# fatimp/SIFT3D

Hardware: AMD Instinct MI355X
Metric: Mvoxel/s detect+describe (float32 volume resident in HBM) (higher is better)
Workload: dtype f32; 1 GPU; 512x512x512 float32 lattice-blob volume, detect+describe, default parameters (sigma0 1.6, sigma_n 1.15, 3 levels/octave); parallelism=single GPU

## Files before the change

profiles/describe_model.py:

```python
#!/usr/bin/env python3
import csv
import glob
import json
import os
import sys

ROOT = os.path.dirname(os.path.dirname(os.path.abspath(__file__)))
sys.path.insert(0, ROOT)


def _require_built():
    lib = os.environ.get("SIFT3D_AMD_LIB") or os.path.join(ROOT, "sift3d_amd", "libsift3d_amd.so")
    if not os.path.exists(lib):
        sys.exit("%s is missing -- build first: python3 -c \"from sift3d_amd import _native; "
                 "_native.build()\"" % lib)


def run_guarded(*a, **k):
    _require_built()
    return run(*a, **k)


def run(n=512):
    import torch
    from sift3d_amd import api, hip
    vol = torch.empty((n, n, n), device="cuda")
    hip.synth_lattice(vol, 0, 11)
    det, kp, desc = api.Detector(), api.KeypointStore(), api.DescriptorStore()
    assert det.detect_keypoints_device(vol.data_ptr(), n, n, n, kp) == 0
    assert det.extract_descriptors(kp, desc) == 0
    return det, kp, desc


def count():
    import ctypes as C
    from sift3d_amd import api
    L = api.lib()
    L.sift3d_amd_diag_desc_voxels.restype = C.c_ulonglong
    L.sift3d_amd_diag_desc_voxels()
    _require_built()
    det, kp, desc = run()
    print(json.dumps(dict(window_voxels=int(L.sift3d_amd_diag_desc_voxels()), keypoints=len(kp))))


def parse(d, voxels):
    agg = {}
    for f in glob.glob(os.path.join(d, "**", "*counter_collection.csv"), recursive=True):
        for r in csv.DictReader(open(f)):
            if "k_describe" in r["Kernel_Name"]:
                agg.setdefault(r["Counter_Name"], []).append(float(r["Counter_Value"]))
    c = {k: sum(v) / len(v) for k, v in agg.items()}
    out = dict(kernel="k_describe", workload="512^3 lattice volume, 42 501 keypoints", window_voxels=int(voxels),
               valu_insts=c.get("SQ_INSTS_VALU"), salu_insts=c.get("SQ_INSTS_SALU"),
               lds_insts=c.get("SQ_INSTS_LDS"), lds_array_cycles=c.get("SQ_LDS_IDX_ACTIVE"),
               lds_bank_conflict_cycles=c.get("SQ_LDS_BANK_CONFLICT"), waves=c.get("SQ_WAVES"),
               wave_quad_cycles=c.get("SQ_WAVE_CYCLES"), wait_any=c.get("SQ_WAIT_ANY"),
               wait_inst_any=c.get("SQ_WAIT_INST_ANY"), wait_inst_lds=c.get("SQ_WAIT_INST_LDS"),
               note="wave-instructions per launch (rocprofv3 --pmc); lds_array_cycles is summed over the 256 CUs; "
                    "bench.py prices both against the kernel's own cycle count of its run (clock probe)")
    if voxels and c.get("SQ_INSTS_VALU"):
        out["valu_insts_per_64_voxels"] = round(64.0 * c["SQ_INSTS_VALU"] / voxels, 1)
        out["lds_insts_per_64_voxels"] = round(64.0 * c.get("SQ_INSTS_LDS", 0) / voxels, 1)
        out["lds_array_cycles_per_64_voxels"] = round(64.0 * c.get("SQ_LDS_IDX_ACTIVE", 0) / voxels, 1)
    if c.get("SQ_WAVE_CYCLES") and c.get("SQ_WAVES"):
        kc = 4.0 * c["SQ_WAVE_CYCLES"] / c["SQ_WAVES"]
        out["profiled_kernel_cycles"] = round(kc)
        out["lds_array_busy"] = round(c.get("SQ_LDS_IDX_ACTIVE", 0) / (256.0 * kc), 4)
        out["valu_busy"] = round(2.0 * c.get("SQ_INSTS_VALU", 0) / (1024.0 * kc), 4)
        if c.get("GRBM_GUI_ACTIVE"):
            out["grbm_gui_active_cycles"] = c["GRBM_GUI_ACTIVE"]
    print(json.dumps(out, indent=1))


if __name__ == "__main__":
    if "--run" in sys.argv:
        run_guarded()
    elif "--count" in sys.argv:
        count()
    elif "--parse" in sys.argv:
        i = sys.argv.index("--parse")
        parse(sys.argv[i + 1], float(sys.argv[i + 2]))
```

sift3d_amd/csrc/sift3d_describe.hip:

```cpp
#include "sift3d_kernels_common.h"
#include "sift3d_math.h"

#include <algorithm>
#include <cmath>
#include <cstdlib>

struct FaceRec {
    float v0[3], e1[3], e2[3], t[3], q[3], e2q, idx[3];
};
static_assert(sizeof(FaceRec) == SIFT3D_HIP_FACE_FLOATS * 4, "face record layout");

__constant__ float c_face16[20 * 16];
__constant__ int c_bin_off[12];
__constant__ int c_oct_face[32];

constexpr int DQ = 256;
constexpr int HIST_USED = 800;
constexpr int HIST_LDS = 800;
constexpr int FACE_STRIDE = 20;
constexpr int RSUPER = 68;
constexpr int REC_FLOATS = 7 * RSUPER;
constexpr int rec_row(int r) { return r < 7 ? r * RSUPER : (r - 7) * RSUPER + 32; }
constexpr int rec_group(int r) { return (rec_row(r) / 4) % 16; }
constexpr bool rec_groups_distinct()
{
    for (int a = 0; a < 14; a++)
        for (int b = a + 1; b < 14; b++)
            if (rec_group(a) == rec_group(b))
                return false;
    return true;
}
static_assert(rec_groups_distinct(), "record rows: X (0..10) and bin-address rows (11..13) on disjoint bank groups");
static_assert(RSUPER % 4 == 0 && RSUPER >= 64, "record rows: 16-byte aligned, 64 lanes per super-row");

__device__ __forceinline__ uint32_t lds_addr(const void *p)
{
    return (uint32_t)(uintptr_t)(const __attribute__((address_space(3))) void *)p;
}

#ifdef SIFT3D_AMD_DIAG
#define DESC_ABLATE_ARG , int ablate
#define DESC_ABLATE(bit) (ablate & (bit))
__device__ unsigned long long g_desc_voxels;
#else
#define DESC_ABLATE_ARG
#define DESC_ABLATE(bit) false
#endif

__device__ __forceinline__ void wave_sync()
{
    __builtin_amdgcn_fence(__ATOMIC_RELEASE, "wavefront");
    __builtin_amdgcn_wave_barrier();
    __builtin_amdgcn_fence(__ATOMIC_ACQUIRE, "wavefront");
}

__device__ __forceinline__ float quad_fmac(float acc, float x)
{
    asm("v_fmac_f32_dpp %0, %1, %1 quad_perm:[3,0,0,0] row_mask:0xf bank_mask:0xf bound_ctrl:1"
        : "+v"(acc)
        : "v"(x));
    return acc;
}

__device__ __forceinline__ bool face_eval(const float4 *__restrict__ fr, float rx, float ry, float rz,
                                          float &xb, float &yb, float &zb, int &fi)
{
    const float4 A0 = fr[0], A1 = fr[1], A2 = fr[2], A3 = fr[3];
    const float px = ry * A1.y - rz * A1.x;
    const float py = rz * A0.w - rx * A1.y;
    const float pz = rx * A1.x - ry * A0.w;
    const float det = A0.x * px + A0.y * py + A0.z * pz;
    const float di = 1.0f / det;
    yb = di * (A1.z * px + A1.w * py + A2.x * pz);
    zb = di * (rx * A2.y + ry * A2.z + rz * A2.w);
    xb = 1.0f - yb - zb;
    const float kk = A3.x * di;
    fi = __float_as_int(A3.y);
    return !(fabsf(det) < 1.1920928955078125e-06f) &&
           !(xb < -1.1920928955078125e-06f || yb < -1.1920928955078125e-06f ||
             zb < -1.1920928955078125e-06f || kk < 0);
}

__device__ __forceinline__ int icos_guess(float rx, float ry, float rz)
{
    const float g = 1.6180339887f, g2 = 2.6180339887f;
    const float ax = fabsf(rx), ay = fabsf(ry), az = fabsf(rz);
    const float t1 = ax + g2 * ay - g * az;
    const float t2 = ay + g2 * az - g * ax;
    const float t3 = az + g2 * ax - g * ay;
    const int n1 = t1 < 0.0f, n2 = t2 < 0.0f, n3 = t3 < 0.0f;
    const int cls = n1 + (1 - n1) * (2 * n2 + (1 - n2) * 3 * n3);
    return cls * 8 + (int)(rx < 0.0f) + 2 * (int)(ry < 0.0f) + 4 * (int)(rz < 0.0f);
}

constexpr int WL_STRIDE = 4096, WL_HEAD = 4;
constexpr int WL_COUNTERS = 16;

__global__ __launch_bounds__(256) void k_desc_wlut(const sift3d_hip_level *__restrict__ levels, int nlevels,
                                                   float *__restrict__ lut)
{
    const int t = blockIdx.x;
    if (t >= nlevels)
        return;
    if (t == 0 && threadIdx.x < WL_COUNTERS)
        reinterpret_cast<uint32_t *>(lut + (size_t)nlevels * WL_STRIDE)[threadIdx.x] = 0u;
    const sift3d_hip_level L = levels[t];
    float *tab = lut + (size_t)t * WL_STRIDE;
    const float sigma = (float)(L.sd * 7.071067812);
    const float rad = (float)(2.0 * (double)sigma);
    const float rad2 = rad * rad, sig2 = sigma * sigma;
    int e;
    const float mant = frexpf(L.ux, &e);
    const float u2 = L.ux * L.ux;
    const bool ok = L.ux == L.uy && L.ux == L.uz && mant == 0.5f &&
                    rad2 / u2 < (float)(WL_STRIDE - WL_HEAD - 1) && u2 * (float)WL_STRIDE < 16777216.0f;
    if (threadIdx.x == 0) {
        tab[0] = ok ? 1.0f : 0.0f;
        tab[1] = 0.0f;
        tab[2] = __int_as_float((int)(__double_as_longlong(L.sd) & 0xffffffffll));
        tab[3] = __int_as_float((int)(__double_as_longlong(L.sd) >> 32));
    }
    if (!ok)
        return;
    for (int k = threadIdx.x; k < WL_STRIDE - WL_HEAD; k += 256) {
        const float sq = (float)k * u2;
        const float arg = -0.5f * sq / sig2;
// ... 39 lines not shown
    if (probe) {
        probe_c0 = clock64();
        probe_w0 = wall_clock64();
    }
    const bool split = !EXACT && part != nullptr;
    for (bool first_pass = true;; first_pass = false) {
    uint32_t item;
    if (work) {
        uint32_t t = 0;
        if (lane == 0)
            t = atomicAdd(work, 1u);
        item = (uint32_t)__builtin_amdgcn_readfirstlane((int)t);
    } else {
        if (!first_pass)
            break;
        item = blockIdx.x * DWAVES + wv;
    }
    const uint32_t ki = first + (split ? item / DPARTS : item);
    const int pp = split ? (int)(item % DPARTS) : 0;
    if (ki >= n)
        break;
    static_assert(2 * HIST_LDS == 25 * 64, "histogram clear: 25 whole-wave stores");
#define Z4(o) "ds_write_addtid_b32 %0 offset:" #o "\n\tds_write_addtid_b32 %0 offset:" #o "+256\n\t" \
              "ds_write_addtid_b32 %0 offset:" #o "+512\n\tds_write_addtid_b32 %0 offset:" #o "+768\n\t"
    asm volatile("s_mov_b32 m0, %1\n\ts_nop 0\n\t" Z4(0) Z4(1024) Z4(2048) Z4(3072) Z4(4096) Z4(5120)
                 "ds_write_addtid_b32 %0 offset:6144" ::"v"(0.0f), "s"(hist_m0) : "m0", "memory");
#undef Z4
    wave_sync();
    const sift3d_hip_kp K = kps[ki];
    const sift3d_hip_level L = levels[K.level];
    const uint32_t orow = K.row1 ? K.row1 - 1 : ki;
    const float *__restrict__ wtab = nullptr;
    const int icx = (int)K.cx, icy = (int)K.cy, icz = (int)K.cz;
    if (LATTICE) {
        wtab = wlut + (size_t)K.level * WL_STRIDE + WL_HEAD;
    } else if (wlut) {
        const float *tab = wlut + (size_t)K.level * WL_STRIDE;
        const long long sdbits = ((long long)__float_as_int(tab[3]) << 32) | (unsigned)__float_as_int(tab[2]);
        if (tab[0] == 1.0f && sdbits == __double_as_longlong(K.sd) && (float)icx == K.cx &&
            (float)icy == K.cy && (float)icz == K.cz)
            wtab = tab + WL_HEAD;
    }

    typedef const float __attribute__((address_space(1))) *gfloat_p;
    const bool have_tab = LATTICE || wtab;
    const gfloat_p wsrc = have_tab ? (gfloat_p)wtab : (gfloat_p) reinterpret_cast<const float *>(levels);
    const int wmask = have_tab ? -1 : 0;

    const float sigma = (float)(K.sd * 7.071067812);
    const float rad = (float)(2.0 * (double)sigma);
    const float half_w = (float)((double)rad / 1.4142135623730951);
    const float desc_w = 2.0f * half_w;
    const float hist_w = desc_w / 4.0f;
    const float bin_f = 1.0f / hist_w;
    const float rad2 = rad * rad;
    const float sig2 = sigma * sigma;
    const float *R = K.R;
    const float iux = 1.0f / L.ux, iuy = 1.0f / L.uy, iuz = 1.0f / L.uz;
    Box B;
    bounds_f(K.cx, rad, L.ux, L.nx, B.xs, B.xe);
    bounds_f(K.cy, rad, L.uy, L.ny, B.ys, B.ye);
    bounds_f(K.cz, rad, L.uz, L.nz_glob, B.zs, B.ze);
    B.zs = max(B.zs, L.z_off + 1);
    B.ze = min(B.ze, L.z_off + L.nz - 2);
    const int xsh = 32 - __builtin_clz((unsigned)max(B.xe - B.xs, 1));
    const int ysh = xsh + 32 - __builtin_clz((unsigned)max(B.ye - B.ys, 1));
    const uint32_t xmask = (1u << xsh) - 1u, ymask = (1u << (ysh - xsh)) - 1u;
#if defined(__HIP_DEVICE_COMPILE__) && !defined(__gfx942__) && !defined(__gfx950__)
#error "k_describe's commit routes its factors with DPP quad_perm on wave64: validated on gfx942 / gfx950 only"
#endif
    const int half = lane >> 5, l5 = lane & 31;
    const int pc = l5 >> 2, pt = l5 & 3, pj = pt < 3 ? pt : 0;
    const int pxr = pt == 0 ? pc : 8 + pj;
    const int pdx = (pc >> 2) & 1, pdy = (pc >> 1) & 1, pdz = pc & 1;
    const int corner4 = 4 * (pdx + 4 * pdy + 16 * pdz);
    const int coff_a = corner4 + (EXACT ? (half == 0 ? 0 : HIST_LDS * 4) : half * (HIST_LDS * 4));
    const int coff_b = corner4 + (half == 1 ? 0 : HIST_LDS * 4);
    (void)coff_b;

    uint32_t qhead = 0, qtail = 0;
    bool pend = false;
#ifdef SIFT3D_AMD_DIAG
    unsigned diag_voxels = 0;
#endif

    auto window = [&](int x, int y, int z, float &sq, float &vbx, float &vby, float &vbz) -> bool {
        const float dx = ((float)x - K.cx) * L.ux;
        const float dy = ((float)y - K.cy) * L.uy;
        const float dz = ((float)z - K.cz) * L.uz;
        sq = dx * dx + dy * dy + dz * dz;
        const float kx = R[0] * dx + R[3] * dy + R[6] * dz;
        const float ky = R[1] * dx + R[4] * dy + R[7] * dz;
        const float kz = R[2] * dx + R[5] * dy + R[8] * dz;
        vbx = (kx + half_w) * bin_f;
        vby = (ky + half_w) * bin_f;
        vbz = (kz + half_w) * bin_f;
        const float lo = fminf(fminf(vbx, vby), vbz), hi = fmaxf(fmaxf(vbx, vby), vbz);
        return !(sq > rad2) && !(lo < 0.0f) && !(hi >= 4.0f);
    };

    float pv[7] = { 0.f, 0.f, 0.f, 0.f, 0.f, 0.f, 0.f };
    int ppk = 0;
    int pwi = 0, pwj = 0, pwl = 0;
    const gfloat_p gdata = (gfloat_p)L.data;
    const uint32_t ys32 = (uint32_t)L.nx, zs32 = (uint32_t)L.nx * (uint32_t)L.ny;
    auto prefetch_loads = [&](uint32_t start, int cnt) {
        const int qv = queue[(start + lane) & (DQ - 1)];
        ppk = lane < cnt ? qv : ppk;
        const int x = B.xs + (int)((uint32_t)ppk & xmask), y = B.ys + (int)(((uint32_t)ppk >> xsh) & ymask),
                  zl = B.zs + (int)((uint32_t)ppk >> ysh) - L.z_off;
        const gfloat_p p = gdata + ((uint64_t)zs32 * (uint32_t)zl + (uint32_t)(x + (int)ys32 * y));
        pv[0] = p[1]; pv[1] = *(p - 1); pv[2] = p[ys32]; pv[3] = *(p - ys32);
        pv[4] = p[zs32]; pv[5] = *(p - zs32);
        if (wtab) {
            const int i = x - icx, j = y - icy, l = B.zs + (int)((uint32_t)ppk >> ysh) - icz;
            pv[6] = wtab[i * i + j * j + l * l];
            pwi = i; pwj = j; pwl = l;
        }
    };
    auto prefetch_weight = [&]() {
        if (LATTICE || wtab)
            return;
        const int x = B.xs + (int)((uint32_t)ppk & xmask), y = B.ys + (int)(((uint32_t)ppk >> xsh) & ymask);
        const float dx = ((float)x - K.cx) * L.ux;
        const float dy = ((float)y - K.cy) * L.uy;
        const float dz = ((float)(B.zs + (int)((uint32_t)ppk >> ysh)) - K.cz) * L.uz;
        pv[6] = s3d_expf_in_range(-0.5f * (dx * dx + dy * dy + dz * dz) / sig2, sexp);
    };
    auto prefetch = [&](uint32_t start, int cnt) {
        prefetch_loads(start, cnt);
        prefetch_weight();
    };

    float rp[2][7] = { { 0.f, 0.f, 0.f, 0.f, 0.f, 0.f, 0.f }, { 0.f, 0.f, 0.f, 0.f, 0.f, 0.f, 0.f } };
    const float *const xrd = rec + rec_row(pxr) + 16 * half;
    const int *const ard = reinterpret_cast<const int *>(rec + rec_row(11 + pj) + 16 * half);
    auto commit_write = [&](int pass) {
#define RS(i) "ds_write_addtid_b32 %" #i " offset:%c8*" #i "\n\t"
        asm volatile("s_mov_b32 m0, %7\n\ts_nop 0\n\t" RS(0) RS(1) RS(2) RS(3) RS(4) RS(5) RS(6)
                     ::"v"(rp[pass][0]), "v"(rp[pass][1]), "v"(rp[pass][2]), "v"(rp[pass][3]), "v"(rp[pass][4]),
                       "v"(rp[pass][5]), "v"(rp[pass][6]), "s"(rec_m0), "n"(RSUPER * 4)
                     : "m0", "memory");
#undef RS
        wave_sync();
    };
#define SB() __builtin_amdgcn_sched_barrier(0)
#ifndef DESC_OPT
#define DESC_OPT 111
#endif
#define QUAD_X(v) __int_as_float(__builtin_amdgcn_update_dpp(0, __float_as_int(v), 0x03, 0xf, 0xf, true))
#if DESC_OPT & 1
#define COMMIT_ADD(old, x) (EXACT ? (old) + QUAD_X(x) * (x) : quad_fmac(old, x))
#else
#define COMMIT_ADD(old, x) ((old) + QUAD_X(x) * (x))
#endif
#define KEEP(v) asm volatile("" ::"v"(v))
#if (DESC_OPT & 64)
typedef __attribute__((address_space(3))) float *lds_float_p;
#define LDS_F32(a) (*(lds_float_p)(uintptr_t)(uint32_t)(a))
#define OFFCHAIN (!EXACT)
#define CHUNK_ADDR(q)                                                                         \
    aq_[q] = make_int4(bq_[q].x + coffh, bq_[q].y + coffh, bq_[q].z + coffh, bq_[q].w + coffh); \
    KEEP(aq_[q].x); KEEP(aq_[q].y); KEEP(aq_[q].z); KEEP(aq_[q].w);
#define COMMIT_BEGIN(coff)                                                                    \
    const int coffh = (coff) + (int)lds_addr(hist);                                           \
    int4 bq_[2], aq_[2];                                                                      \
    float4 xq_[2];                                                                            \
    bq_[0] = *reinterpret_cast<const int4 *>(ard);                                            \
    xq_[0] = *reinterpret_cast<const float4 *>(xrd);                                          \
    bq_[1] = bq_[0];                                                                          \
    xq_[1] = xq_[0];                                                                          \
    CHUNK_ADDR(0)                                                                             \
    aq_[1] = aq_[0];
#define ROUND(u, ...)                                                                         \
    {                                                                                         \
        constexpr int cur_ = ((u) >> 2) & 1, nxt_ = cur_ ^ 1;                                 \
        const int mb_[4] = { bq_[cur_].x, bq_[cur_].y, bq_[cur_].z, bq_[cur_].w };            \
        const int ma_[4] = { aq_[cur_].x, aq_[cur_].y, aq_[cur_].z, aq_[cur_].w };            \
        const float xv_[4] = { xq_[cur_].x, xq_[cur_].y, xq_[cur_].z, xq_[cur_].w };          \
        const int addr_ = OFFCHAIN ? ma_[(u) & 3] : mb_[(u) & 3] + coffh;                     \
        float old_ = 0.0f;                                                                    \
        if (!DESC_ABLATE(1))                                                                  \
            old_ = LDS_F32(addr_);                                                            \
        SB();                                                                                 \
        if (((u) & 3) == 0 && (u) + 4 < 16) {                                                 \
            bq_[nxt_] = *reinterpret_cast<const int4 *>(ard + (u) + 4);                       \
            xq_[nxt_] = *reinterpret_cast<const float4 *>(xrd + (u) + 4);                     \
            SB();                                                                             \
        }                                                                                     \
        { __VA_ARGS__ }                                                                       \
        if (OFFCHAIN && ((u) & 3) == 1 && (u) + 3 < 16) {                                     \
            CHUNK_ADDR(nxt_)                                                                  \
        }                                                                                     \
        SB();                                                                                 \
        if (!DESC_ABLATE(1))                                                                  \
            LDS_F32(addr_) = COMMIT_ADD(old_, xv_[(u) & 3]);            \
        SB();                                                                                 \
    }
#else
#define COMMIT_BEGIN(coff)                                                                    \
    const int coff4 = (coff);                                                                 \
    int4 cb4 = *reinterpret_cast<const int4 *>(ard);                                          \
    float4 cx4 = *reinterpret_cast<const float4 *>(xrd);                                      \
    int4 nb4 = cb4;                                                                           \
    float4 nx4 = cx4;
#define ROUND(u, ...)                                                                         \
    {                                                                                         \
        if (((u) & 3) == 0 && (u) + 4 < 16) {                                                 \
            nb4 = *reinterpret_cast<const int4 *>(ard + (u) + 4);                             \
            nx4 = *reinterpret_cast<const float4 *>(xrd + (u) + 4);                           \
        }                                                                                     \
        const int mb_[4] = { cb4.x, cb4.y, cb4.z, cb4.w };                                    \
        const float xv_[4] = { cx4.x, cx4.y, cx4.z, cx4.w };                                  \
        float *bin_ = reinterpret_cast<float *>(reinterpret_cast<char *>(hist) + (mb_[(u) & 3] + coff4)); \
        float old_ = 0.0f;                                                                    \
        if (!DESC_ABLATE(1))                                                                  \
            old_ = *bin_;                                                                     \
        SB();                                                                                 \
        { __VA_ARGS__ }                                                                       \
        SB();                                                                                 \
        if (!DESC_ABLATE(1))                                                                  \
            *bin_ = COMMIT_ADD(old_, xv_[(u) & 3]);                     \
        if (((u) & 3) == 3) {                                                                 \
            cb4 = nb4;                                                                        \
            cx4 = nx4;                                                                        \
        }                                                                                     \
        SB();                                                                                 \
    }
#endif
#define CHAIN_B()                                                                             \
    if (EXACT) {                                                                              \
// ... 92 lines not shown
            float mag, fx, fy, fz;
            int ix, iy, iz, cell4;
            float ax[2], ay[2], az[2], fld[14];
            ROUND(0, qv_ = queue[(nstart + lane) & (DQ - 1)];)
            ROUND(1, ppk = lane < ncnt ? qv_ : ppk;
                     nx_ = B.xs + (int)((uint32_t)ppk & xmask); ny_ = B.ys + (int)(((uint32_t)ppk >> xsh) & ymask);
                     nzl_ = B.zs + (int)((uint32_t)ppk >> ysh) - L.z_off;
                     np_ = gdata + ((uint64_t)zs32 * (uint32_t)nzl_ + (uint32_t)(nx_ + (int)ys32 * ny_));)
            ROUND(2, pv[0] = np_[1]; pv[1] = *(np_ - 1); pv[2] = np_[ys32]; pv[3] = *(np_ - ys32);)
            ROUND(3, pv[4] = np_[zs32]; pv[5] = *(np_ - zs32);
                     const int i = nx_ - icx; const int j = ny_ - icy; const int l = B.zs + (int)((uint32_t)ppk >> ysh) - icz;
                     pv[6] = wsrc[(i * i + j * j + l * l) & wmask];
                     if (LATTICE && (DESC_OPT & 8)) { pwi = i; pwj = j; pwl = l; })
#if DESC_OPT & 2
            ROUND(4, mag = EXACT ? sqrtf(m2) : __builtin_amdgcn_sqrtf(m2);
                     mag = live && found ? mag : 0.0f;)
#else
            ROUND(4, mag = sqrtf(m2); mag = live && found ? mag : 0.0f;)
#endif
            ROUND(5, fx = vbx - floorf(vbx); fy = vby - floorf(vby); fz = vbz - floorf(vbz);
                     ix = (int)vbx; iy = (int)vby; iz = (int)vbz;)
            ROUND(6, const bool lx = ix >= 3; const bool ly = iy >= 3; const bool lz = iz >= 3;
                     ax[0] = lx ? 0.0f : 1.0f - fx; ax[1] = lx ? 1.0f - fx : fx;
                     ay[0] = ly ? 0.0f : 1.0f - fy; ay[1] = ly ? 1.0f - fy : fy;
                     az[0] = lz ? 0.0f : 1.0f - fz; az[1] = lz ? 1.0f - fz : fz;)
            ROUND(7, _Pragma("unroll") for (int c = 0; c < 4; c++)
                         fld[c] = mag * (ax[(c >> 2) & 1] * ay[(c >> 1) & 1] * az[c & 1]);)
            ROUND(8, _Pragma("unroll") for (int c = 4; c < 8; c++)
                         fld[c] = mag * (ax[(c >> 2) & 1] * ay[(c >> 1) & 1] * az[c & 1]);)
            ROUND(9, cell4 = 4 * (min(max(ix, 0), 2) + 4 * min(max(iy, 0), 2) + 16 * min(max(iz, 0), 2));
                     const bool ok = live && found;
                     fld[8] = ok ? b0 : 0.0f; fld[9] = ok ? b1 : 0.0f; fld[10] = ok ? b2 : 0.0f;)
            ROUND(10, _Pragma("unroll") for (int j = 0; j < 3; j++)
                          fld[11 + j] = __int_as_float(4 * ((fidx >> (10 * j)) & 1023) + cell4);)
            ROUND(11, _Pragma("unroll") for (int i = 0; i < 4; i++) {
                          const auto r = __builtin_amdgcn_permlane32_swap(__float_as_uint(fld[i]), __float_as_uint(fld[7 + i]), false, false);
                          rp[0][i] = __uint_as_float(r[0]); rp[1][i] = __uint_as_float(r[1]); })
            ROUND(12, _Pragma("unroll") for (int i = 4; i < 7; i++) {
                          const auto r = __builtin_amdgcn_permlane32_swap(__float_as_uint(fld[i]), __float_as_uint(fld[7 + i]), false, false);
                          rp[0][i] = __uint_as_float(r[0]); rp[1][i] = __uint_as_float(r[1]); })
            ROUND(13, )
            ROUND(14, )
            ROUND(15, )
        }
        CHAIN_B();
        prefetch_weight();
    };
    auto commit_tail = [&](int pass) {
        commit_write(pass);
        {
            COMMIT_BEGIN(coff_a);
            ROUND(0, ) ROUND(1, ) ROUND(2, ) ROUND(3, ) ROUND(4, ) ROUND(5, ) ROUND(6, ) ROUND(7, )
            ROUND(8, ) ROUND(9, ) ROUND(10, ) ROUND(11, ) ROUND(12, ) ROUND(13, ) ROUND(14, ) ROUND(15, )
        }
        CHAIN_B();
    };

    float ortho = 0.0f;
#pragma unroll
    for (int a = 0; a < 3; a++)
#pragma unroll
        for (int b = a; b < 3; b++)
            ortho = fmaxf(ortho, fabsf(R[a] * R[b] + R[3 + a] * R[3 + b] + R[6 + a] * R[6 + b] - (a == b ? 1.0f : 0.0f)));
    const bool cube_ok = ortho <= 1e-4f;
    const float cube_x = cube_ok ? half_w * (fabsf(R[0]) + fabsf(R[1]) + fabsf(R[2])) * 1.001f : rad * 1.001f;
    const float cube_y = cube_ok ? half_w * (fabsf(R[3]) + fabsf(R[4]) + fabsf(R[5])) * 1.001f : rad * 1.001f;
    const float cube_z = cube_ok ? half_w * (fabsf(R[6]) + fabsf(R[7]) + fabsf(R[8])) * 1.001f : rad * 1.001f;
    int zs = max(B.zs, (int)floorf(K.cz - cube_z / L.uz - 1.0f));
    int ze = min(B.ze, (int)ceilf(K.cz + cube_z / L.uz + 1.0f));
    if (split) {
        const int np_ = max(ze - zs + 1, 0);
        const int c1 = (33 * np_ + 50) / 100, c2 = (np_ + 1) / 2, c3 = (67 * np_ + 50) / 100;
        static_assert(DPARTS == 4, "three cuts");
        const int lo = pp == 0 ? 0 : pp == 1 ? c1 : pp == 2 ? c2 : c3;
        const int hi = pp == 0 ? c1 : pp == 1 ? c2 : pp == 2 ? c3 : np_;
        ze = zs + hi - 1;
        zs = zs + lo;
    }
#if DESC_OPT & 4
    const float wa0 = R[0] * L.ux * bin_f, wa1 = R[1] * L.ux * bin_f, wa2 = R[2] * L.ux * bin_f;
    const float wb0 = R[3] * L.uy * bin_f, wb1 = R[4] * L.uy * bin_f, wb2 = R[5] * L.uy * bin_f;
    const float rad2_in = rad2 * 0.9999f, rad2_out = rad2 * 1.0001f;
#endif
    for (int z = zs; z <= ze; z++) {
        const float dzp = ((float)z - K.cz) * L.uz;
        const float rz = sqrtf(fmaxf(rad2 - dzp * dzp, 0.0f)) * 1.001f;
        const float xr = fminf(rz, cube_x) / L.ux + 1.0f, yr = fminf(rz, cube_y) / L.uy + 1.0f;
        const int pxs = max(B.xs, (int)floorf(K.cx - xr)), pxe = min(B.xe, (int)ceilf(K.cx + xr));
        const int pys = max(B.ys, (int)floorf(K.cy - yr)), pye = min(B.ye, (int)ceilf(K.cy + yr));
        const int pbx = pxe - pxs + 1, pby = pye - pys + 1;
        const int ox = pxs - B.xs, oy = pys - B.ys;
#if DESC_OPT & 4
        const float dx0 = ((float)pxs - K.cx) * L.ux, dy0 = ((float)pys - K.cy) * L.uy, dz2 = dzp * dzp;
        const float wc0 = (R[0] * dx0 + R[3] * dy0 + R[6] * dzp + half_w) * bin_f;
        const float wc1 = (R[1] * dx0 + R[4] * dy0 + R[7] * dzp + half_w) * bin_f;
        const float wc2 = (R[2] * dx0 + R[5] * dy0 + R[8] * dzp + half_w) * bin_f;
        auto cheap2 = [&](int xx_, int yy_, bool &acc0, bool &acc1) -> bool {
            const float fx_ = (float)xx_, fy_ = (float)yy_, gx_ = (float)(xx_ + 1);
            const float t0 = __builtin_fmaf(wb0, fy_, wc0), t1 = __builtin_fmaf(wb1, fy_, wc1),
                        t2 = __builtin_fmaf(wb2, fy_, wc2);
            const float ey = __builtin_fmaf(fy_, L.uy, dy0), sy = __builtin_fmaf(ey, ey, dz2);
            const float v0 = __builtin_fmaf(wa0, fx_, t0), v1 = __builtin_fmaf(wa1, fx_, t1),
                        v2 = __builtin_fmaf(wa2, fx_, t2);
            const float u0 = __builtin_fmaf(wa0, gx_, t0), u1 = __builtin_fmaf(wa1, gx_, t1),
                        u2 = __builtin_fmaf(wa2, gx_, t2);
            const float ex = __builtin_fmaf(fx_, L.ux, dx0), fx2 = __builtin_fmaf(gx_, L.ux, dx0);
            const float sq_ = __builtin_fmaf(ex, ex, sy), sq2 = __builtin_fmaf(fx2, fx2, sy);
            const float lo = fminf(fminf(v0, v1), v2), hi = fmaxf(fmaxf(v0, v1), v2);
            const float lo2 = fminf(fminf(u0, u1), u2), hi2 = fmaxf(fmaxf(u0, u1), u2);
            acc0 = sq_ <= rad2_in && lo >= 1e-4f && hi <= 3.9999f;
            acc1 = sq2 <= rad2_in && lo2 >= 1e-4f && hi2 <= 3.9999f;
            const bool rej0 = sq_ > rad2_out || lo < -1e-4f || hi >= 4.0001f;
            const bool rej1 = sq2 > rad2_out || lo2 < -1e-4f || hi2 >= 4.0001f;
            return (!acc0 && !rej0) || (!acc1 && !rej1);
        };
#endif
        const int pbe = pbx + (pbx & 1);
        const int ppe = pbx > 0 && pby > 0 ? pbe * pby : 0;
        const int q128 = pbe > 0 ? 128 / pbe : 0, r128 = pbe > 0 ? 128 - q128 * pbe : 0;
        int yy = pbe > 0 ? (2 * lane) / pbe : 0, xx = pbe > 0 ? 2 * lane - yy * pbe : 0;
        for (int c0 = 0; c0 < ppe; c0 += 128) {
#if DESC_OPT & 4
            bool in0, in1;
            if (__builtin_expect(__ballot(cheap2(xx, yy, in0, in1)) != 0ull, 0)) {
                float sq, vbx, vby, vbz;
                in0 = window(pxs + xx, pys + yy, z, sq, vbx, vby, vbz);
                in1 = window(pxs + xx + 1, pys + yy, z, sq, vbx, vby, vbz);
            }
#else
            float sq, vbx, vby, vbz;
            bool in0 = window(pxs + xx, pys + yy, z, sq, vbx, vby, vbz);
            bool in1 = window(pxs + xx + 1, pys + yy, z, sq, vbx, vby, vbz);
#endif
            in0 = in0 && c0 + 2 * lane < ppe;
            in1 = in1 && c0 + 2 * lane < ppe && xx + 1 < pbx;
            const int pk0 = (int)((uint32_t)(ox + xx) | ((uint32_t)(oy + yy) << xsh) | ((uint32_t)(z - B.zs) << ysh));
            const int pk1 = pk0 + 1;
            xx += r128;
            yy += q128;
            if (xx >= pbe) {
                xx -= pbe;
                yy++;
            }
            const unsigned long long m0 = __ballot(in0), m1 = __ballot(in1);
            if ((m0 | m1) == 0ull)
                continue;
#if DESC_OPT & 32
            const uint32_t before = __builtin_amdgcn_mbcnt_hi(
                (uint32_t)(m1 >> 32), __builtin_amdgcn_mbcnt_lo((uint32_t)m1, __builtin_amdgcn_mbcnt_hi(
                (uint32_t)(m0 >> 32), __builtin_amdgcn_mbcnt_lo((uint32_t)m0, 0u))));
#else
            const unsigned long long lt_mask = (1ull << lane) - 1ull;
            const uint32_t before = (uint32_t)__popcll(m0 & lt_mask) + (uint32_t)__popcll(m1 & lt_mask);
#endif
            if (in0)
                queue[(qtail + before) & (DQ - 1)] = pk0;
            if (in1)
                queue[(qtail + before + (in0 ? 1u : 0u)) & (DQ - 1)] = pk1;
            qtail += (uint32_t)__popcll(m0) + (uint32_t)__popcll(m1);
            wave_sync();
            while (qtail - qhead >= 64) {
                if (pend) {
                    float cv[7];
#pragma unroll
                    for (int k = 0; k < 7; k++)
                        cv[k] = pv[k];
                    const int cpk = ppk;
                    batch(64, cv, cpk, qhead, 64);
                } else {
                    prefetch(qhead, 64);
                    pend = true;
                }
                qhead += 64;
            }
        }
    }
    {
        int have = pend ? 64 : 0, rest = (int)(qtail - qhead);
        if (!have && rest) {
            prefetch(qhead, rest);
            have = rest;
            rest = 0;
        }
        while (have) {
            float cv[7];
#pragma unroll
            for (int k = 0; k < 7; k++)
                cv[k] = pv[k];
            const int cpk = ppk, cnt = have;
            batch(cnt, cv, cpk, qhead, rest);
            have = rest;
            rest = 0;
        }
    }
#ifdef SIFT3D_AMD_DIAG
    if (lane == 0)
        atomicAdd(&g_desc_voxels, (unsigned long long)diag_voxels);
#endif
    commit_tail(0);
    commit_tail(1);
    wave_sync();
    const float trunc = 0.2f * 128.0f / 768.0f;
    if (!EXACT) {
        for (int i = lane; i < HIST_USED; i += 64)
            hist[i] = hist[i] + hist[HIST_LDS + i];
        wave_sync();
    }
    if (split) {
        float *mine = part + ((size_t)(ki - first) * DPARTS + (size_t)pp) * HIST_USED;
        for (int i = lane; i < HIST_USED; i += 64)
            __hip_atomic_store(mine + i, hist[i], __ATOMIC_RELAXED, __HIP_MEMORY_SCOPE_AGENT);
        asm volatile("s_waitcnt vmcnt(0)" ::: "memory");
        uint32_t arrived = 0;
        if (lane == 0)
            arrived = __hip_atomic_fetch_add(done + (ki - first), 1u, __ATOMIC_RELAXED, __HIP_MEMORY_SCOPE_AGENT);
        arrived = (uint32_t)__builtin_amdgcn_readfirstlane((int)arrived);
        if (arrived != DPARTS - 1) {
            wave_sync();
            continue;
        }
        const float *all = part + (size_t)(ki - first) * DPARTS * HIST_USED;
        for (int i = lane; i < HIST_USED; i += 64) {
            float v = __hip_atomic_load(all + i, __ATOMIC_RELAXED, __HIP_MEMORY_SCOPE_AGENT);
#pragma unroll
            for (int q = 1; q < DPARTS; q++)
                v = v + __hip_atomic_load(all + (size_t)q * HIST_USED + i, __ATOMIC_RELAXED, __HIP_MEMORY_SCOPE_AGENT);
            hist[i] = v;
        }
        wave_sync();
    }
    for (int pass = 0; pass < 2; pass++) {
        double norm = 0.0;
        if (EXACT) {
            for (int c = 0; c < 64; c++)
#pragma unroll
                for (int b = 0; b < 12; b++) {
                    const float el = hist[c_bin_off[b] + c];
                    norm += (double)el * (double)el;
                }
        } else {
            for (int i = lane; i < HIST_USED; i += 64) {
                const float el = hist[i];
                norm += (double)el * (double)el;
            }
#pragma unroll
            for (int o = 32; o > 0; o >>= 1)
                norm += __shfl_xor(norm, o, 64);
        }
        norm = sqrt(norm) + 2.220446049250313e-16;
        const float inv = (float)(1.0 / norm);
        wave_sync();
        for (int i = lane; i < HIST_USED; i += 64) {
            float el = hist[i] * inv;
            if (pass == 0)
                el = el < trunc ? el : trunc;
            hist[i] = el;
        }
        wave_sync();
    }
    for (int i = lane; i < 768; i += 64) {
        const float v = hist[c_bin_off[i % 12] + i / 12];
        out[(size_t)orow * 768 + i] = v;
        if (out2)
            out2[(size_t)orow * 768 + i] = v;
    }
    wave_sync();
    }
    if (probe) {
        unsigned long long *slot =
            reinterpret_cast<unsigned long long *>(work - (EXACT ? 0 : LATTICE ? 2 : 1) + (EXACT ? 4 : 8));
        slot[0] = (unsigned long long)(clock64() - probe_c0);
        slot[1] = (unsigned long long)(wall_clock64() - probe_w0);
    }
}

__constant__ int c_face_vert[20];

constexpr int DB_TX = 64, DB_TY = 4;

__device__ __forceinline__ void dense_bin_one(const float *sface, const int *soct, const int *svert, float gx,
// ... 438 lines not shown
                if (colour[u] == c)
                    binoff[u] = 64 * rank++ + shift[c];
    }
    for (int f = 0; f < 20; f++) {
        const int packed = binoff[idx[f * 3]] | (binoff[idx[f * 3 + 1]] << 10) |
                           (binoff[idx[f * 3 + 2]] << 20);
        memcpy(f16 + f * 16 + 13, &packed, sizeof(int));
    }
    int oct[32];
    {
        const float g = 1.6180339887f;
        const float rep[4][3] = { { 1.0f, 1.0f, 1.0f },
                                  { g / 3.0f, 0.05f, (2.0f * g + 1.0f) / 3.0f },
                                  { (2.0f * g + 1.0f) / 3.0f, g / 3.0f, 0.05f },
                                  { 0.05f, (2.0f * g + 1.0f) / 3.0f, g / 3.0f } };
        for (int c = 0; c < 4; c++)
            for (int o = 0; o < 8; o++) {
                const float r[3] = { (o & 1) ? -rep[c][0] : rep[c][0], (o & 2) ? -rep[c][1] : rep[c][1],
                                     (o & 4) ? -rep[c][2] : rep[c][2] };
                int hit = -1;
                for (int f = 0; f < 20 && hit < 0; f++)
                    if (host_face_pass(f16, f, r))
                        hit = f;
                if (hit < 0) {
                    snprintf(g_err, sizeof(g_err), "sift3d_hip_set_mesh: no face holds a probe direction");
                    return SIFT3D_FAILURE;
                }
                oct[c * 8 + o] = hit;
            }
    }
    HIPCHK(hipMemcpyToSymbol(HIP_SYMBOL(c_bin_off), binoff, sizeof(binoff)));
    HIPCHK(hipMemcpyToSymbol(HIP_SYMBOL(c_face16), f16, sizeof(f16)));
    HIPCHK(hipMemcpyToSymbol(HIP_SYMBOL(c_oct_face), oct, sizeof(oct)));
    int vert[20];
    {
        float P[20][3][3];
        for (int f = 0; f < 20; f++)
            for (int k = 0; k < 3; k++) {
                const float *r = faces + f * SIFT3D_HIP_FACE_FLOATS;
                P[f][0][k] = r[k];
                P[f][1][k] = r[k] + r[3 + k];
                P[f][2][k] = r[k] + r[6 + k];
            }
        auto near = [&](const float *a, int g) {
            for (int j = 0; j < 3; j++)
                if (fabsf(a[0] - P[g][j][0]) + fabsf(a[1] - P[g][j][1]) + fabsf(a[2] - P[g][j][2]) < 1e-3f)
                    return true;
            return false;
        };
        for (int f = 0; f < 20; f++) {
            vert[f] = 0;
            for (int j = 0; j < 3; j++) {
                int id = -1;
                for (int a = 0; a < 3 && id < 0; a++) {
                    bool all = true;
                    for (int g = 0; g < 20; g++)
                        for (int b = 0; b < 3; b++)
                            if (idx[g * 3 + b] == idx[f * 3 + a])
                                all = all && near(P[f][j], g);
                    if (all)
                        id = idx[f * 3 + a];
                }
                if (id < 0) {
                    snprintf(g_err, sizeof(g_err), "sift3d_hip_set_mesh: face %d has no vertex id for corner %d", f, j);
                    return SIFT3D_FAILURE;
                }
                vert[f] |= id << (4 * j);
            }
        }
    }
    HIPCHK(hipMemcpyToSymbol(HIP_SYMBOL(c_face_vert), vert, sizeof(vert)));
    return SIFT3D_SUCCESS;
}

#ifdef SIFT3D_AMD_DIAG
__attribute__((visibility("default"))) unsigned long long sift3d_amd_diag_desc_voxels(void)
{
    unsigned long long v = 0, z = 0;
    (void)hipDeviceSynchronize();
    (void)hipMemcpyFromSymbol(&v, HIP_SYMBOL(g_desc_voxels), sizeof(v));
    (void)hipMemcpyToSymbol(HIP_SYMBOL(g_desc_voxels), &z, sizeof(z));
    return v;
}
#endif

size_t sift3d_hip_describe_wlut_floats(int nlevels)
{
    return nlevels > 0 ? (size_t)nlevels * WL_STRIDE + WL_COUNTERS : 0;
}

static unsigned describe_grid(uint32_t count, bool counted)
{
    const unsigned need = (count + DWAVES - 1) / DWAVES;
    if (!counted)
        return need;
    static int cus = 0;
    if (!cus) {
        int dev = 0;
        hipDeviceProp_t prop;
        if (hipGetDevice(&dev) == hipSuccess && hipGetDeviceProperties(&prop, dev) == hipSuccess)
            cus = prop.multiProcessorCount;
        if (cus < 1)
            cus = 256;
    }
    const unsigned cap = (unsigned)cus * 4u;
    return need < cap ? need : cap;
}

size_t sift3d_hip_describe_part_bytes(uint32_t n)
{
    return n ? (size_t)n * DPARTS * HIST_USED * sizeof(float) + (size_t)n * sizeof(uint32_t) : 0;
}

int sift3d_hip_describe_lattice_level(float ux, float uy, float uz, double sd)
{
    const float sigma = (float)(sd * 7.071067812);
    const float rad = (float)(2.0 * (double)sigma);
    int e;
    const float mant = frexpf(ux, &e);
    const float rad2 = rad * rad, u2 = ux * ux;
    return ux == uy && ux == uz && mant == 0.5f && ux >= 0.0009765625f && ux <= 1024.0f &&
           rad2 / u2 < 0.999f * (float)(WL_STRIDE - WL_HEAD - 1) && u2 * (float)WL_STRIDE < 16777216.0f;
}

static int describe_launch(const sift3d_hip_level *d_levels, int nlevels, const sift3d_hip_kp *d_kp, uint32_t n,
                           uint32_t n_exact, uint32_t n_lattice, float *d_hist, float *d_hist2,
                           const float *d_wlut, void *d_part, void *stream)
{
    if (n_exact > n)
        n_exact = n;
    if (!(DESC_OPT & 8) || !d_wlut)
        n_lattice = 0;
    if (n_lattice > n - n_exact)
        return launch_fail("sift3d_hip_describe", "more lattice records than fast records");
#ifdef SIFT3D_AMD_DIAG
    static int ablate = getenv("SIFT3D_AMD_DESC_ABLATE") ? atoi(getenv("SIFT3D_AMD_DESC_ABLATE")) : 0;
#define DESC_ABLATE_PASS , ablate
#else
#define DESC_ABLATE_PASS
#endif
    uint32_t *work = d_wlut ? reinterpret_cast<uint32_t *>(const_cast<float *>(d_wlut) + (size_t)nlevels * WL_STRIDE)
                            : nullptr;
    if (n_exact) {
        hipLaunchKernelGGL(k_describe<true>, dim3(describe_grid(n_exact, work != nullptr)), dim3(64 * DWAVES), 0,
                           (hipStream_t)stream, d_levels, d_kp, 0u, n_exact, d_hist, d_hist2, d_wlut,
                           work, (float *)nullptr, (uint32_t *)nullptr DESC_ABLATE_PASS);
        LAUNCH_CHECK();
    }
    if (n > n_exact) {
        const uint32_t nf = n - n_exact;
        void *tmp = nullptr;
        if (!d_part) {
            HIPCHK(hipMalloc(&tmp, sift3d_hip_describe_part_bytes(nf)));
            d_part = tmp;
        }
        float *parts = reinterpret_cast<float *>(d_part);
        uint32_t *done = reinterpret_cast<uint32_t *>(parts + (size_t)nf * DPARTS * HIST_USED);
        hipError_t e = hipMemsetAsync(done, 0, (size_t)nf * sizeof(uint32_t), (hipStream_t)stream);
        const uint32_t ng = nf - n_lattice;
        if (e == hipSuccess && ng) {
            hipLaunchKernelGGL((k_describe<false, false>), dim3(describe_grid(ng * DPARTS, work != nullptr)),
                               dim3(64 * DWAVES), 0, (hipStream_t)stream, d_levels, d_kp, n_exact, n - n_lattice,
                               d_hist, d_hist2, d_wlut, work ? work + 1 : nullptr, parts, done DESC_ABLATE_PASS);
            e = hipGetLastError();
        }
        if (e == hipSuccess && n_lattice) {
// ... 201 lines not shown
```

Measured before the change: 4431 Mvoxel/s.

## Tighten describe per-plane scan footprint with rotated-cube cross-section bounding box

Enables a new DESC_OPT bit (128). Per z-plane, the scan rectangle is now intersected with the bounding box of the rotated descriptor cube's cross-section in that plane, computed from edge/plane intersections. Lanes compute the boxes for 64 planes at once, and each plane reads its box back with readlane. The aim is to test fewer voxels that the window predicate would reject anyway, at the cost of extra per-plane setup math plus margin heuristics that must keep every accepted voxel inside the box. Diagnostic counters for tested positions and a footprint-model script are added as well.

```diff
diff --git a/profiles/describe_model.py b/profiles/describe_model.py
--- a/profiles/describe_model.py
+++ b/profiles/describe_model.py
@@ -37,10 +37,14 @@
     from sift3d_amd import api
     L = api.lib()
     L.sift3d_amd_diag_desc_voxels.restype = C.c_ulonglong
+    L.sift3d_amd_diag_desc_tested.restype = C.c_ulonglong
     L.sift3d_amd_diag_desc_voxels()
+    L.sift3d_amd_diag_desc_tested()
     _require_built()
     det, kp, desc = run()
-    print(json.dumps(dict(window_voxels=int(L.sift3d_amd_diag_desc_voxels()), keypoints=len(kp))))
+    voxels, tested = int(L.sift3d_amd_diag_desc_voxels()), int(L.sift3d_amd_diag_desc_tested())
+    print(json.dumps(dict(window_voxels=voxels, tested_positions=tested,
+                          tested_per_surviving=round(tested / max(voxels, 1), 4), keypoints=len(kp))))
 
 
 def parse(d, voxels):
diff --git a/profiles/microbench/scan_footprint_model.py b/profiles/microbench/scan_footprint_model.py
--- /dev/null
+++ b/profiles/microbench/scan_footprint_model.py
@@ -0,0 +1,45 @@
+#!/usr/bin/env python3
+import os
+import sys
+
+import numpy as np
+
+ROOT = os.path.dirname(os.path.dirname(os.path.dirname(os.path.abspath(__file__))))
+sys.path.insert(0, ROOT)
+
+from tests.test_describe_scan_footprint_host import Window
+
+
+def main():
+    g = np.load(os.path.join(ROOT, "tests", "golden", "g5_512.npz"), allow_pickle=False)
+    n0 = int(g["dims"][0])
+    tot = dict(acc=0, rect=0, box=0, exact=0, exact2=0)
+    used = fallback = 0
+    for (o, _), (x, y, z, sd), R in zip(g["kp_os_s"], g["kp_xyzsd_s"], g["kp_R_s"]):
+        w = Window((x, y, z), sd, R, n=n0 >> int(o), u=2.0 ** int(o))
+        ext = float(w.rad / w.u)
+        if min(x, y, z) - ext < 2 or max(x, y, z) + ext > (n0 >> int(o)) - 3:
+            continue
+        used += 1
+        zz = w.planes()
+        acc = w.accepted(zz)
+        tot["acc"] += int(acc.sum())
+        for name, (xs, xe, ys, ye) in (("rect", w.plane_rect(zz)), ("box", w.plane_box(zz))):
+            tot[name] += int((np.maximum(xe - xs + 1, 0) * np.maximum(ye - ys + 1, 0)).sum())
+        fallback += all(np.array_equal(a, b) for a, b in zip(w.plane_rect(zz), w.plane_box(zz)))
+        for p in range(len(zz)):
+            ys, xs = np.nonzero(acc[p])
+            if len(xs):
+                wx, wy = xs.max() - xs.min() + 1, ys.max() - ys.min() + 1
+                tot["exact"] += int(wx * wy)
+                tot["exact2"] += int((wx + 4) * (wy + 4))
+    print("%d of %d sampled keypoints have interior windows; %d of them keep plane_rect in every plane" %
+          (used, len(g["kp_os_s"]), fallback))
+    print("%-12s %18s %28s" % ("footprint", "tested / surviving", "128-chunks per 64-voxel batch"))
+    for name, key in (("plane_rect", "rect"), ("plane_box", "box"), ("exact", "exact"), ("exact + 2", "exact2")):
+        r = tot[key] / tot["acc"]
+        print("%-12s %18.3f %28.3f" % (name, r, r / 2.0))
+
+
+if __name__ == "__main__":
+    main()
diff --git a/sift3d_amd/csrc/sift3d_describe.hip b/sift3d_amd/csrc/sift3d_describe.hip
--- a/sift3d_amd/csrc/sift3d_describe.hip
+++ b/sift3d_amd/csrc/sift3d_describe.hip
@@ -42,6 +42,7 @@
 #define DESC_ABLATE_ARG , int ablate
 #define DESC_ABLATE(bit) (ablate & (bit))
 __device__ unsigned long long g_desc_voxels;
+__device__ unsigned long long g_desc_tested;
 #else
 #define DESC_ABLATE_ARG
 #define DESC_ABLATE(bit) false
@@ -247,6 +248,7 @@
     bool pend = false;
 #ifdef SIFT3D_AMD_DIAG
     unsigned diag_voxels = 0;
+    unsigned diag_tested = 0;
 #endif
 
     auto window = [&](int x, int y, int z, float &sq, float &vbx, float &vby, float &vbz) -> bool {
@@ -311,7 +313,7 @@
     };
 #define SB() __builtin_amdgcn_sched_barrier(0)
 #ifndef DESC_OPT
-#define DESC_OPT 111
+#define DESC_OPT 239
 #endif
 #define QUAD_X(v) __int_as_float(__builtin_amdgcn_update_dpp(0, __float_as_int(v), 0x03, 0xf, 0xf, true))
 #if DESC_OPT & 1
@@ -570,12 +572,69 @@
     const float wb0 = R[3] * L.uy * bin_f, wb1 = R[4] * L.uy * bin_f, wb2 = R[5] * L.uy * bin_f;
     const float rad2_in = rad2 * 0.9999f, rad2_out = rad2 * 1.0001f;
 #endif
+    auto plane_rect = [&](float dzp, int &pxs, int &pxe, int &pys, int &pye) {
+        const float rz = sqrtf(fmaxf(rad2 - dzp * dzp, 0.0f)) * 1.001f;
+        const float xr = fminf(rz, cube_x) / L.ux + 1.0f, yr = fminf(rz, cube_y) / L.uy + 1.0f;
+        pxs = max(B.xs, (int)floorf(K.cx - xr)), pxe = min(B.xe, (int)ceilf(K.cx + xr));
+        pys = max(B.ys, (int)floorf(K.cy - yr)), pye = min(B.ye, (int)ceilf(K.cy + yr));
+    };
+#if DESC_OPT & 128
+    auto plane_box = [&](int zl, uint32_t &wx, uint32_t &wy) {
+        float r[9], hw = half_w;
+#pragma unroll
+        for (int k = 0; k < 9; k++)
+            r[k] = R[k];
+        asm volatile("" : "+v"(r[0]), "+v"(r[1]), "+v"(r[2]), "+v"(r[3]), "+v"(r[4]), "+v"(r[5]), "+v"(r[6]),
+                          "+v"(r[7]), "+v"(r[8]), "+v"(hw));
+        const bool poly_ok = cube_ok && fminf(fminf(fabsf(r[0] * r[4] - r[1] * r[3]), fabsf(r[0] * r[5] - r[2] * r[3])),
+                                              fabsf(r[1] * r[5] - r[2] * r[4])) >= 1e-2f;
+        const float dz = ((float)zl - K.cz) * L.uz;
+        float hx = -__builtin_inff(), lx = __builtin_inff(), hy = hx, ly = lx;
+#pragma unroll
+        for (int pr = 0; pr < 3; pr++) {
+            const int i = pr == 2 ? 1 : 0, j = pr == 0 ? 1 : 2, k = 3 - i - j;
+            const float idet = __builtin_amdgcn_rcpf(r[i] * r[3 + j] - r[j] * r[3 + i]);
+#pragma unroll
+            for (int sg = 0; sg < 4; sg++) {
+                const float p = ((sg & 1) ? -hw : hw) - r[6 + i] * dz, q = ((sg & 2) ? -hw : hw) - r[6 + j] * dz;
+                const float vx = (p * r[3 + j] - q * r[3 + i]) * idet, vy = (r[i] * q - r[j] * p) * idet;
+                const bool ok = fabsf(r[k] * vx + r[3 + k] * vy + r[6 + k] * dz) <= hw * 1.001f;
+                hx = ok ? fmaxf(hx, vx) : hx;
+                lx = ok ? fminf(lx, vx) : lx;
+                hy = ok ? fmaxf(hy, vy) : hy;
+                ly = ok ? fminf(ly, vy) : ly;
+            }
+        }
+        int pxs, pxe, pys, pye;
+        plane_rect(dz, pxs, pxe, pys, pye);
+        if (poly_ok && hx >= lx && hy >= ly) {
+            const float mg = hw * 0.0015f;
+            pxs = max(pxs, (int)floorf(K.cx + (lx - mg) * iux - 1.0f));
+            pxe = min(pxe, (int)ceilf(K.cx + (hx + mg) * iux + 1.0f));
+            pys = max(pys, (int)floorf(K.cy + (ly - mg) * iuy - 1.0f));
+            pye = min(pye, (int)ceilf(K.cy + (hy + mg) * iuy + 1.0f));
+        }
+        wx = min((uint32_t)(pxs - B.xs), 65535u) | (min((uint32_t)(B.xe - pxe), 65535u) << 16);
+        wy = min((uint32_t)(pys - B.ys), 65535u) | (min((uint32_t)(B.ye - pye), 65535u) << 16);
+    };
+    uint32_t boxx = 0, boxy = 0;
+#endif
     for (int z = zs; z <= ze; z++) {
         const float dzp = ((float)z - K.cz) * L.uz;
-        const float rz = sqrtf(fmaxf(rad2 - dzp * dzp, 0.0f)) * 1.001f;
-        const float xr = fminf(rz, cube_x) / L.ux + 1.0f, yr = fminf(rz, cube_y) / L.uy + 1.0f;
-        const int pxs = max(B.xs, (int)floorf(K.cx - xr)), pxe = min(B.xe, (int)ceilf(K.cx + xr));
-        const int pys = max(B.ys, (int)floorf(K.cy - yr)), pye = min(B.ye, (int)ceilf(K.cy + yr));
+#if DESC_OPT & 128
+        if (z == zs || (z & 63) == 0)
+            plane_box((z & ~63) + lane, boxx, boxy);
+        const uint32_t wx = (uint32_t)__builtin_amdgcn_readlane((int)boxx, z & 63);
+        const uint32_t wy = (uint32_t)__builtin_amdgcn_readlane((int)boxy, z & 63);
+        const int pxs = B.xs + (int)(wx & 65535u), pxe = B.xe - (int)(wx >> 16);
+        const int pys = B.ys + (int)(wy & 65535u), pye = B.ye - (int)(wy >> 16);
+#else
+        int pxs, pxe, pys, pye;
+        plane_rect(dzp, pxs, pxe, pys, pye);
+#endif
+#ifdef SIFT3D_AMD_DIAG
+        diag_tested += (unsigned)(max(pxe - pxs + 1, 0) * max(pye - pys + 1, 0));
+#endif
         const int pbx = pxe - pxs + 1, pby = pye - pys + 1;
         const int ox = pxs - B.xs, oy = pys - B.ys;
 #if DESC_OPT & 4
@@ -684,6 +743,8 @@
 #ifdef SIFT3D_AMD_DIAG
     if (lane == 0)
         atomicAdd(&g_desc_voxels, (unsigned long long)diag_voxels);
+    if (lane == 0)
+        atomicAdd(&g_desc_tested, (unsigned long long)diag_tested);
 #endif
     commit_tail(0);
     commit_tail(1);
@@ -1288,6 +1349,15 @@
     (void)hipMemcpyToSymbol(HIP_SYMBOL(g_desc_voxels), &z, sizeof(z));
     return v;
 }
+
+__attribute__((visibility("default"))) unsigned long long sift3d_amd_diag_desc_tested(void)
+{
+    unsigned long long v = 0, z = 0;
+    (void)hipDeviceSynchronize();
+    (void)hipMemcpyFromSymbol(&v, HIP_SYMBOL(g_desc_tested), sizeof(v));
+    (void)hipMemcpyToSymbol(HIP_SYMBOL(g_desc_tested), &z, sizeof(z));
+    return v;
+}
 #endif
 
 size_t sift3d_hip_describe_wlut_floats(int nlevels)
```

Result: no change. 4468 Mvoxel/s, median of 6 (+0.8%).
